# KrishnaswamyLab/MELD

Hardware: AMD Instinct MI355X
Metric: cells/sec through MELD.fit_transform (kNN+Chebyshev) (higher is better)
Workload: dtype f64

## Files before the change

### meld_amd/csrc/knn16.hip

```cpp
#include "common.hpp"

#include <hip/hip_fp16.h>

#include <algorithm>

namespace meld {

constexpr int K16_TS = 64;
constexpr int K16_BQ = 256;
constexpr int K16_THREADS = 256;
constexpr int K16_NWAVE = K16_THREADS / 64;
constexpr int K16_SLACK = 128;
constexpr int K16_CAPMAX = 256;
constexpr int K16_BOUNDS_THREADS = 1024;
constexpr int K16_SLOTS = K16_CAPMAX / 64;
constexpr int K16_DMAX = 16 * 9 - 3;

constexpr int K16_SPLIT_DA = 13;
__host__ __device__ inline void k16_slot(int c, int d, int dA, int* coord, int* piece) {
  *coord = -1;
  *piece = -1;
  if (dA == 0) {
    if (c < d) *coord = c;
    else if (c < d + 3) *piece = 3 + (c - d);
    return;
  }
  const int nb = d - dA;
  if (c < dA) *coord = c;
  else if (c < dA + 3) *piece = c - dA;
  else if (c < 16) return;
  else if (c < 16 + nb) *coord = dA + (c - 16);
  else if (c < 16 + nb + 3) *piece = 3 + (c - 16 - nb);
}

typedef float f32x16 __attribute__((ext_vector_type(16)));
typedef _Float16 f16x8 __attribute__((ext_vector_type(8)));

__device__ __forceinline__ float min3f(float a, float b, float c) { return __builtin_fminf(__builtin_fminf(a, b), c); }
__device__ __forceinline__ float min16(const f32x16& v) {
  const float a = min3f(v[0], v[1], v[2]);
  const float b = min3f(v[3], v[4], v[5]);
  const float c = min3f(v[6], v[7], v[8]);
  const float d = min3f(v[9], v[10], v[11]);
  const float e = min3f(v[12], v[13], v[14]);
  return __builtin_fminf(min3f(a, b, v[15]), min3f(c, d, e));
}

__device__ __forceinline__ unsigned ordered_bits(float f) {
  const unsigned b = __float_as_uint(f);
  return (b & 0x80000000u) ? ~b : (b | 0x80000000u);
}

__device__ __forceinline__ float ld_sc1_f(const float* p) {
  return __hip_atomic_load(p, __ATOMIC_RELAXED, __HIP_MEMORY_SCOPE_AGENT);
}
__device__ __forceinline__ int ld_sc1_i(const int* p) {
  return __hip_atomic_load(p, __ATOMIC_RELAXED, __HIP_MEMORY_SCOPE_AGENT);
}

#define K16_COLD_REGION_END() __builtin_amdgcn_s_waitcnt(0x0F70)

__device__ __forceinline__ bool knn16_row_slot(int p, int n0, int n1, int half, int* q) {
  if (p < half) {
    *q = p;
    return p < n0;
  }
  *q = n0 + (p - half);
  return (p - half) < n1;
}
__device__ __forceinline__ int knn16_split_pos(int pos, int m0, int half) { return pos < m0 ? pos : half + (pos - m0); }

__device__ __forceinline__ float from_ordered_bits(unsigned k) {
  return __uint_as_float((k & 0x80000000u) ? (k & 0x7fffffffu) : ~k);
}

__device__ float knn16_squeeze_row(int n0, int n1, int half, int ksel, int knn1, float rf2, float err, float nq_row,
                                   float* __restrict__ d2row, int* __restrict__ idxrow, int lane, int* n0_out,
                                   int* n1_out, float* r_out) {
  asm volatile("s_waitcnt vmcnt(0)" ::: "memory");
  float d[K16_SLOTS];
  int ix[K16_SLOTS];
  unsigned key[K16_SLOTS];
  bool valid[K16_SLOTS];
#pragma unroll
  for (int e = 0; e < K16_SLOTS; ++e) {
    const int p = lane + 64 * e;
    int q;
    valid[e] = p < 2 * half && knn16_row_slot(p, n0, n1, half, &q);
    if (valid[e]) {
      d[e] = ld_sc1_f(d2row + p);
      ix[e] = ld_sc1_i(idxrow + p);
      key[e] = ordered_bits(d[e]);
    } else {
      d[e] = INFINITY;
      ix[e] = 0x7fffffff;
      key[e] = 0xffffffffu;
    }
  }
  unsigned T = 0;
#pragma unroll 1
  for (int bit = 31; bit >= 0; --bit) {
    const unsigned trial = T | (1u << bit);
    int c = 0;
#pragma unroll
    for (int e = 0; e < K16_SLOTS; ++e) c += __popcll(__ballot(key[e] < trial));
    if (c < ksel) T = trial;
  }
  float R = INFINITY;
  if (knn1 > 0 && n0 + n1 >= knn1) {
    unsigned A = 0;
#pragma unroll 1
    for (int bit = 31; bit >= 0; --bit) {
      const unsigned trial = A | (1u << bit);
      int c = 0;
#pragma unroll
      for (int e = 0; e < K16_SLOTS; ++e) c += __popcll(__ballot(key[e] < trial));
      if (c < knn1) A = trial;
    }
    R = (rf2 * ((from_ordered_bits(A) + nq_row) + err) + err) * 1.00001f + 1e-30f - nq_row;
  }
  *r_out = R;
  const unsigned Tc = min(T, ordered_bits(R));
  int total = 0;
#pragma unroll
  for (int e = 0; e < K16_SLOTS; ++e) total += __popcll(__ballot(valid[e] && key[e] <= Tc));
  const int m0 = (total + 1) >> 1;
  int base = 0;
  float thr = INFINITY;
#pragma unroll
  for (int e = 0; e < K16_SLOTS; ++e) {
    const bool keep = valid[e] && key[e] <= Tc;
    const unsigned long long b = __ballot(keep);
    if (keep) {
      const int dst = knn16_split_pos(base + __popcll(b & ((1ull << lane) - 1ull)), m0, half);
      d2row[dst] = d[e];
      idxrow[dst] = ix[e];
    }
    base += __popcll(b);
    const unsigned long long bt = __ballot(valid[e] && key[e] == T);
    if (bt) thr = __shfl(d[e], __ffsll((long long)bt) - 1, 64);
  }
  *n0_out = m0;
  *n1_out = total - m0;
  return thr;
}

__device__ void knn16_rank_row(int n0, int n1, int half, int ksel, float out_scale, float add, int split_m0,
                               float* __restrict__ d2row, int* __restrict__ idxrow, float* sd, int* si, int lane) {
  asm volatile("s_waitcnt vmcnt(0)" ::: "memory");
  const int n = n0 + n1;
  float d[K16_SLOTS];
  int ix[K16_SLOTS];
  bool valid[K16_SLOTS];
#pragma unroll
  for (int e = 0; e < K16_SLOTS; ++e) {
    const int p = lane + 64 * e;
    int q = 0;
    valid[e] = p < 2 * half && knn16_row_slot(p, n0, n1, half, &q);
    if (valid[e]) {
      d[e] = ld_sc1_f(d2row + p);
      ix[e] = ld_sc1_i(idxrow + p);
      sd[q] = d[e];
      si[q] = ix[e];
    } else {
      d[e] = INFINITY;
      ix[e] = 0x7fffffff;
    }
  }
  asm volatile("s_waitcnt lgkmcnt(0)" ::: "memory");
  int rk[K16_SLOTS];
#pragma unroll
  for (int q = 0; q < K16_SLOTS; ++q) rk[q] = 0;
  for (int e = 0; e < n; ++e) {
    const float de = sd[e];
    const int ie = si[e];
#pragma unroll
    for (int q = 0; q < K16_SLOTS; ++q) rk[q] += (de < d[q] || (de == d[q] && ie < ix[q])) ? 1 : 0;
  }
#pragma unroll
  for (int q = 0; q < K16_SLOTS; ++q) {
    if (valid[q] && rk[q] < ksel) {
      const int dst = split_m0 < 0 ? rk[q] : knn16_split_pos(rk[q], split_m0, half);
      d2row[dst] = (d[q] + add) * out_scale;
      idxrow[dst] = ix[q];
    }
  }
  asm volatile("s_waitcnt lgkmcnt(0)" ::: "memory");
}

__device__ __forceinline__ int k16_scan_tile(int s, int t0, int n_scan, int two_sided) {
  int off = s;
  if (two_sided && s >= K16_BQ / K16_TS) {
    const int j = s - K16_BQ / K16_TS;
    off = (j & 1) ? -1 - (j >> 1) : K16_BQ / K16_TS + (j >> 1);
  }
  const int t = t0 + off;
  return t >= n_scan ? t - n_scan : (t < 0 ? t + n_scan : t);
}

struct K16Args {
  const _Float16* Q16;
  const float* Qn;
  const _Float16* Rt16;
  const float* scale_info;
  int n_ref, n_tiles, ksel, cap;
  const __half* lb2;
  const float* norm2_max;
  float err_coef;
  int tile_origin, batch_every, batch_slack, two_sided;
  unsigned long long* stats;
  const float* thr_init;
  int knn1;
  float rf2, err_c, err_l;
  int* cand_idx;
  float* cand_d2;
  int* cand_cnt;
  float* cand_thr;
  unsigned long long* tiles_done;
  const int* block_order;
  const unsigned* step_list;
  const int* step_cnt;
  long long list_stride;
  int ee_hi;
  int planes_used;
  int count_go;
};
#define K16_COLD(FIELD) \
  (((const volatile K16Args __attribute__((address_space(4)))*)__builtin_amdgcn_kernarg_segment_ptr())->FIELD)

__host__ __device__ constexpr int k16_waves(int KB, int NPROD, bool EE) {
  return ((NPROD == 1 && KB <= 4) ? 3 : ((KB <= 5 || (NPROD == 1 && KB <= 8)) ? 2 : 1)) + ((EE && KB <= 4) ? 1 : 0);
}

template <int KB, int STATS, int NPROD, bool LIST = false, bool EE = false>
__global__ __launch_bounds__(K16_THREADS)
__attribute__((amdgpu_waves_per_eu(k16_waves(KB, NPROD, EE), k16_waves(KB, NPROD, EE)))) void knn16_topk_kernel(const K16Args a) {
  const _Float16* __restrict__ Q16 = a.Q16;
  const float* __restrict__ Qn = a.Qn;
  const _Float16* __restrict__ Rt16 = a.Rt16;
  const int n_tiles = a.n_tiles, ksel = a.ksel, cap = a.cap;
  const __half* __restrict__ lb2 = LIST ? nullptr : a.lb2;
  const int batch_every = a.batch_every, two_sided = a.two_sided;
  int* __restrict__ cand_idx = a.cand_idx;
  float* __restrict__ cand_d2 = a.cand_d2;
  constexpr int TILE_H = KB * 2 * 2 * K16_TS * 8;
  constexpr int TILE_V4 = TILE_H / 8;
  constexpr int LDS_TILE_H = (NPROD == 3) ? TILE_H : TILE_H / 2;
  constexpr bool PAIR = EE;
  constexpr int NBUF = PAIR ? 4 : 3;
  __shared__ __attribute__((aligned(16))) _Float16 lds_ring[NBUF * LDS_TILE_H];
  constexpr int TILE_LDS_BYTES = LDS_TILE_H * 2;
  __shared__ float lds_sd[K16_NWAVE][K16_CAPMAX];
  __shared__ int lds_si[K16_NWAVE][K16_CAPMAX];
  unsigned long long (*lds_wlive)[K16_NWAVE];
  if constexpr (!LIST) {
    __shared__ unsigned long long lds_wlive_own[3][K16_NWAVE];
    lds_wlive = lds_wlive_own;
  } else {
    lds_wlive = reinterpret_cast<unsigned long long (*)[K16_NWAVE]>(&lds_sd[0][0]);
  }

  const int tid = threadIdx.x;
  const int lane = tid & 63;
  const int wave = __builtin_amdgcn_readfirstlane(tid >> 6);
  const int jq = lane & 31;
  const int h = lane >> 5;
  const int bx = a.block_order ? __builtin_amdgcn_readfirstlane(a.block_order[blockIdx.y]) : (int)blockIdx.y;
  const int q_base = bx * K16_BQ + wave * 64;
  int sl_n_ = (int)gridDim.x;
  asm volatile("" : "+s"(sl_n_));
  const int sl_n = sl_n_, sl_y = (int)blockIdx.x;
  typedef const __attribute__((address_space(4))) unsigned* k16_list_ptr;
  const k16_list_ptr my_list = LIST ? (k16_list_ptr)(uintptr_t)(a.step_list + (size_t)bx * (size_t)a.list_stride) : (k16_list_ptr)0;
  const int n_scan = ((LIST ? __builtin_amdgcn_readfirstlane(a.step_cnt[bx]) : n_tiles) - sl_y + sl_n - 1) / sl_n;
  auto list_entry = [&](int s_) __attribute__((always_inline)) { return s_ < n_scan ? my_list[sl_y + sl_n * s_] : 0u; };
  auto entry_live = [&](unsigned e) __attribute__((always_inline)) { return ((e >> (24 + wave)) & 1u) != 0u; };
  const int row_base = (int)(blockIdx.x * (gridDim.y * K16_BQ)) + q_base;
  float* const wave_d2 = cand_d2 + (size_t)row_base * cap;
  int* const wave_idx = cand_idx + (size_t)row_base * cap;

  f16x8 bhi[2][KB], blo[2][KB];
#pragma unroll
  for (int g = 0; g < 2; ++g) {
    const f16x8* qrow = reinterpret_cast<const f16x8*>(Q16 + (size_t)(q_base + g * 32 + jq) * (KB * 32));
#pragma unroll
    for (int kb = 0; kb < KB; ++kb) {
      bhi[g][kb] = qrow[(kb * 2 + h) * 2 + 0];
      if (NPROD == 3) blo[g][kb] = qrow[(kb * 2 + h) * 2 + 1];
    }
  }
  const float* const wave_qn = Qn + q_base;

  int cnt[2] = {0, 0};
  const int half = cap >> 1;
  if (!LIST && lane == 0) lds_wlive[0][wave] = lds_wlive[1][wave] = lds_wlive[2][wave] = ~0ull;
  auto thr_start = [&](int g) __attribute__((always_inline)) { return a.thr_init ? a.thr_init[q_base + g * 32 + jq] : INFINITY; };
  float thrp[2] = {thr_start(0) - wave_qn[jq], thr_start(1) - wave_qn[32 + jq]};
  float ee_c[2] = {0.0f, 0.0f};
  if constexpr (EE) {
    const int ee_hi = a.ee_hi;
    const float s_ = a.scale_info[0];
    const float delta = 3.814697265625e-06f * (a.norm2_max[0] * s_ * s_) + 1e-30f;
#pragma unroll
    for (int g = 0; g < 2; ++g) {
      float qb = 0.0f;
#pragma unroll
      for (int kb = 1; kb < KB; ++kb) {
#pragma unroll
        for (int e = 0; e < 8; ++e) {
          const float v = (16 * kb + 8 * h + e < ee_hi) ? (float)bhi[g][kb][e] : 0.0f;
          qb = fmaf(v, v, qb);
        }
      }
      qb += __shfl_xor(qb, 32, 64);
      ee_c[g] = qb * 1.0001f + delta;
    }
  }
  float wmax = INFINITY;
  if (a.thr_init) {
    float w = fmaxf(thr_start(0), thr_start(1));
#pragma unroll
    for (int off = 32; off > 0; off >>= 1) w = fmaxf(w, __shfl_xor(w, off, 64));
    wmax = w;
  }
  unsigned st_go = 0;
  unsigned st_slow = 0, st_app = 0, st_sq = 0;
  unsigned tm_seg = 0, tm_sel = 0, tm_tail = 0, tm_dma = 0, tm_bar = 0, tm_idle = 0, tm_mark = 0;
  auto tm_now = [&]() __attribute__((always_inline)) { return STATS ? (unsigned)__builtin_readcyclecounter() : 0u; };
  auto tm_lap = [&](unsigned& acc) __attribute__((always_inline)) {
    if (STATS) {
      const unsigned n = tm_now();
      acc += n - tm_mark;
      tm_mark = n;
    }
  };

  const float prune_margin = lb2 ? a.err_coef * a.norm2_max[0] * a.scale_info[0] * a.scale_info[0] : 0.0f;
  const int t0 = (int)((((long long)a.tile_origin + (long long)bx * (K16_BQ / K16_TS)) / sl_n) % n_scan);
  const __half* my_lb = lb2 ? lb2 + (size_t)(bx * K16_NWAVE + wave) * n_tiles : nullptr;
  auto tile_of = [&](int s) { return k16_scan_tile(s, t0, n_scan, two_sided) * sl_n + sl_y; };
  int win_base = 0;
  float win_lb = 0.0f;
  unsigned long long win_rem = 0, my_live = ~0ull;
  auto load_window = [&](int base) __attribute__((always_inline)) {
    const int ss = base + lane;
    win_base = base;
    win_lb = ss < n_scan ? __half2float(my_lb[tile_of(ss)]) : INFINITY;
    win_rem = __ballot(ss < n_scan);
    asm volatile("" : "+v"(win_lb));
  };
  if (my_lb) {
    load_window(0);
    win_rem &= ~1ull;
  }
  auto lds_union = [&](int buf) __attribute__((always_inline)) {
    unsigned lo = 0, hi = 0;
#pragma unroll
    for (int w = 0; w < K16_NWAVE; ++w) {
      const uint2 v = *reinterpret_cast<const uint2*>(&lds_wlive[buf][w]);
      lo |= v.x;
      hi |= v.y;
    }
    return ((unsigned long long)(unsigned)__builtin_amdgcn_readfirstlane((int)hi) << 32) |
           (unsigned long long)(unsigned)__builtin_amdgcn_readfirstlane((int)lo);
  };

  const float4* R4 = reinterpret_cast<const float4*>(Rt16);
  int r4_lo_v, r4_hi_v;
  asm volatile("v_mov_b32 %0, %2\n\tv_mov_b32 %1, %3"
               : "=v"(r4_lo_v), "=v"(r4_hi_v)
               : "s"((int)(unsigned)reinterpret_cast<size_t>(R4)), "s"((int)(reinterpret_cast<size_t>(R4) >> 32)));
  constexpr int N_STAGE = (NPROD == 3) ? KB * 256 : KB * 128;
  constexpr int NS = (N_STAGE + K16_THREADS - 1) / K16_THREADS;
  constexpr bool STAGE_TAIL = (N_STAGE % K16_THREADS) != 0;
  static_assert(NS <= 9, "tile too large for the staging rounds");
  const int stage_off = (NPROD == 3) ? tid : (((tid >> 6) << 7) + (tid & 63));
  constexpr int STAGE_STRIDE = (NPROD == 3) ? K16_THREADS : 2 * K16_THREADS;
  const bool stage_last = !STAGE_TAIL || wave < (N_STAGE % K16_THREADS) / 64;
  const int tail_plane = (NS - 1) * (K16_THREADS / 64) + wave;
  const bool skip_tail = NPROD == 1 && NS >= 2 && tail_plane < 2 * KB && tail_plane >= a.planes_used;
  if (skip_tail) {
#pragma unroll
    for (int b = 0; b < NBUF; ++b)
      reinterpret_cast<float4*>(lds_ring + b * LDS_TILE_H)[((NS - 1) * (K16_THREADS / 64) + wave) * 64 + lane] = make_float4(0.f, 0.f, 0.f, 0.f);
  }
#define K16_ROUND_OK(U) (((U) + 1 < NS || stage_last) && !((U) + 1 == NS && skip_tail))
  const int stage_voff = stage_off * 16;
  typedef __attribute__((address_space(3))) void* lds_ptr_t;
  typedef int k16_i32x4 __attribute__((ext_vector_type(4)));
  const unsigned ring_addr = (unsigned)(size_t)(lds_ptr_t)lds_ring + (unsigned)wave * 1024u;
#define K16_DMA(U, DSTB)                                                                                              \
  asm volatile("s_mov_b32 m0, %0\n\ts_nop 0\n\tbuffer_load_dwordx4 %1, %2, %3 offen lds" ::"s"(__builtin_amdgcn_readfirstlane(    \
                   (int)(ring_addr + (DSTB) + (unsigned)((U) * K16_THREADS * 16)))),                                   \
               "v"(stage_voff), "s"(rsrc), "s"((U) * STAGE_STRIDE * 16)                                                \
               : "memory")
#define K16_LOAD(TILE, DSTB)                                                                                       \
  do {                                                                                                             \
    const size_t src_ = (((size_t)(unsigned)__builtin_amdgcn_readfirstlane(r4_hi_v) << 32) |                       \
                         (size_t)(unsigned)__builtin_amdgcn_readfirstlane(r4_lo_v)) +                              \
                        (size_t)(TILE) * (TILE_V4 * 16);                                                           \
    const k16_i32x4 rsrc = {(int)(unsigned)src_, (int)((src_ >> 32) & 0xffffu), TILE_V4 * 16, 0x00020000};         \
    if constexpr (NS > 0) if (K16_ROUND_OK(0)) K16_DMA(0, DSTB);                                                   \
    if constexpr (NS > 1) if (K16_ROUND_OK(1)) K16_DMA(1, DSTB);                                                   \
    if constexpr (NS > 2) if (K16_ROUND_OK(2)) K16_DMA(2, DSTB);                                                   \
    if constexpr (NS > 3) if (K16_ROUND_OK(3)) K16_DMA(3, DSTB);                                                   \
    if constexpr (NS > 4) if (K16_ROUND_OK(4)) K16_DMA(4, DSTB);                                                   \
    if constexpr (NS > 5) if (K16_ROUND_OK(5)) K16_DMA(5, DSTB);                                                   \
    if constexpr (NS > 6) if (K16_ROUND_OK(6)) K16_DMA(6, DSTB);                                                   \
    if constexpr (NS > 7) if (K16_ROUND_OK(7)) K16_DMA(7, DSTB);                                                   \
    if constexpr (NS > 8) if (K16_ROUND_OK(8)) K16_DMA(8, DSTB);                                                   \
  } while (0)
#define K16_STAGED() __builtin_amdgcn_s_waitcnt(0x0F70)
  constexpr int N_INFLIGHT = NS - (STAGE_TAIL ? 1 : 0);
  constexpr int N_INFLIGHT_SKIP = (!STAGE_TAIL && NS >= 2) ? N_INFLIGHT - 1 : N_INFLIGHT;
#define K16_STAGED_BUT_LAST()                                                                                      \
  do {                                                                                                             \
    if (skip_tail) __builtin_amdgcn_s_waitcnt(0x0F70 | (N_INFLIGHT_SKIP & 15) | ((N_INFLIGHT_SKIP >> 4) << 14));   \
    else __builtin_amdgcn_s_waitcnt(0x0F70 | (N_INFLIGHT & 15) | ((N_INFLIGHT >> 4) << 14));                       \
  } while (0)
#define K16_TILE_BARRIER() asm volatile("s_waitcnt lgkmcnt(0)\n\ts_barrier" ::: "memory")
  if constexpr (!PAIR) K16_LOAD(__builtin_amdgcn_readfirstlane(LIST ? (int)(list_entry(0) & 0xFFFFFFu) : tile_of(0)), 0u);

#pragma unroll
  for (int g = 0; g < 2; ++g) {
#pragma unroll
    for (int kb = 0; kb < KB; ++kb) {
      asm volatile("" : "+v"(bhi[g][kb]));
      if (NPROD == 3) asm volatile("" : "+v"(blo[g][kb]));
    }
    asm volatile("" : "+v"(thrp[g]));
  }

  f32x16 accA0, accA1, accB0, accB1;
#pragma unroll
  for (int r = 0; r < 16; ++r) accB0[r] = accB1[r] = INFINITY;
  int refB = 0;

  auto mfma_block = [&](const _Float16* tile, int sub, f32x16& c0, f32x16& c1) __attribute__((always_inline)) {
#pragma unroll
    for (int r = 0; r < 16; ++r) c0[r] = c1[r] = 0.0f;
    const f16x8* a8 = reinterpret_cast<const f16x8*>(tile) + sub * 32 + jq;
#pragma unroll
    for (int kb = 0; kb < KB; ++kb) {
      const f16x8 ahi = NPROD == 3 ? a8[((kb * 2 + h) * 2 + 0) * K16_TS] : a8[(kb * 2 + h) * K16_TS];
      c0 = __builtin_amdgcn_mfma_f32_32x32x16_f16(ahi, bhi[0][kb], c0, 0, 0, 0);
      c1 = __builtin_amdgcn_mfma_f32_32x32x16_f16(ahi, bhi[1][kb], c1, 0, 0, 0);
      if (NPROD == 3) {
        const f16x8 alo = a8[((kb * 2 + h) * 2 + 1) * K16_TS];
        c0 = __builtin_amdgcn_mfma_f32_32x32x16_f16(ahi, blo[0][kb], c0, 0, 0, 0);
        c1 = __builtin_amdgcn_mfma_f32_32x32x16_f16(ahi, blo[1][kb], c1, 0, 0, 0);
        c0 = __builtin_amdgcn_mfma_f32_32x32x16_f16(alo, bhi[0][kb], c0, 0, 0, 0);
        c1 = __builtin_amdgcn_mfma_f32_32x32x16_f16(alo, bhi[1][kb], c1, 0, 0, 0);
      }
    }
  };
  auto vote = [&](const f32x16& c0, const f32x16& c1, float& m0, float& m1) __attribute__((always_inline)) {
    m0 = min16(c0);
    m1 = min16(c1);
  };
  auto squeeze = [&](int g, int j) __attribute__((always_inline)) {
    const int cg = g ? cnt[1] : cnt[0];
    const int n0 = __shfl(cg, j, 64), n1 = __shfl(cg, j + 32, 64);
    const size_t ro = (size_t)(g * 32 + j) * cap;
    int m0, m1;
    float rcut = INFINITY, err = 0.0f;
    const int knn1 = K16_COLD(knn1);
    const float nq_row = wave_qn[g * 32 + j];
    if (knn1 > 0) {
      const float* sinfo = K16_COLD(scale_info);
      const float nmax_s = K16_COLD(norm2_max)[0] * sinfo[0] * sinfo[0];
      err = (K16_COLD(err_c) * nmax_s + K16_COLD(err_l) * sqrtf(nq_row * nmax_s)) * 1.001f;
    }
    float nt = knn16_squeeze_row(n0, n1, half, ksel, knn1, K16_COLD(rf2), err, nq_row, wave_d2 + ro, wave_idx + ro, lane, &m0, &m1, &rcut);
    if (m0 > half - 32) {
      knn16_rank_row(m0, m1, half, ksel, 1.0f, 0.0f, (min(m0 + m1, ksel) + 1) >> 1, wave_d2 + ro, wave_idx + ro, lds_sd[wave],
                     lds_si[wave], lane);
      const int tot = min(m0 + m1, ksel);
      m0 = (tot + 1) >> 1;
      m1 = tot - m0;
      asm volatile("s_waitcnt vmcnt(0)" ::: "memory");
      nt = ld_sc1_f(wave_d2 + ro + knn16_split_pos(tot - 1, m0, half));
    }
    if (jq == j) {
      const int mine = h ? m1 : m0;
      if (g) cnt[1] = mine; else cnt[0] = mine;
      const float t_list = (n0 + n1 >= ksel) ? nt : INFINITY;
      thrp[g] = fminf(thrp[g], fminf(t_list, rcut));
    }
    asm volatile("" : "+v"(thrp[0]), "+v"(thrp[1]), "+v"(cnt[0]), "+v"(cnt[1]));
  };
  auto refresh_wmax = [&]() __attribute__((always_inline)) {
    if (my_lb == nullptr) return;
    float w = fmaxf(thrp[0] + wave_qn[jq], thrp[1] + wave_qn[32 + jq]);
#pragma unroll
    for (int off = 32; off > 0; off >>= 1) w = fmaxf(w, __shfl_xor(w, off, 64));
    wmax = w;
  };
  auto select = [&](const f32x16& c0, const f32x16& c1, float m0, float m1, int ref_base) __attribute__((always_inline)) {
    unsigned long long need = 0;
    if (STATS) ++st_slow;
#pragma unroll
    for (int g = 0; g < 2; ++g) {
      const f32x16 acc = g ? c1 : c0;
      if (!__any((g ? m1 : m0) < thrp[g])) continue;
      const unsigned rowoff4 = (unsigned)((g * 32 + jq) * cap + h * half) * 4u;
      auto append = [&](int r) __attribute__((always_inline)) {
        const float v = acc[r];
        if (v < thrp[g]) {
          const unsigned off4 = rowoff4 + 4u * (unsigned)(g ? cnt[1]++ : cnt[0]++);
          if (STATS) ++st_app;
          *reinterpret_cast<float*>(reinterpret_cast<char*>(wave_d2) + off4) = v;
          *reinterpret_cast<int*>(reinterpret_cast<char*>(wave_idx) + off4) = ref_base + (r & 3) + 8 * (r >> 2);
        }
      };
#pragma unroll
      for (int t = 0; t < 5; ++t) {
        if (__any(min3f(acc[3 * t], acc[3 * t + 1], acc[3 * t + 2]) < thrp[g])) {
          append(3 * t);
          append(3 * t + 1);
          append(3 * t + 2);
        }
      }
      if (__any(acc[15] < thrp[g])) append(15);
      const unsigned long long full = __ballot((g ? cnt[1] : cnt[0]) > half - 16);
      need |= ((full | (full >> 32)) & 0xffffffffull) << (32 * g);
    }
    if (__builtin_expect(need != 0, 0)) {
      while (need) {
        const int j = __ffsll((long long)need) - 1;
        need &= need - 1;
        squeeze(j >> 5, j & 31);
        if (STATS) ++st_sq;
      }
      refresh_wmax();
      K16_COLD_REGION_END();
    }
  };
  constexpr int N_MFMA = 2 * KB * (NPROD == 3 ? 3 : 1);
  constexpr int N_DSR = KB * (NPROD == 3 ? 2 : 1);
  constexpr int VALU_PER_MFMA = (N_MFMA >= 16) ? 1 : ((N_MFMA >= 8) ? 2 : 4);
  auto pipeline_order = [&]() __attribute__((always_inline)) {
    if (NPROD == 3) {
      __builtin_amdgcn_sched_group_barrier(0x100, N_DSR, 0);
      __builtin_amdgcn_sched_group_barrier(0x002, 4, 0);
#pragma unroll
      for (int i = 0; i < N_MFMA; ++i) {
        __builtin_amdgcn_sched_group_barrier(0x008, 1, 0);
        __builtin_amdgcn_sched_group_barrier(0x002, VALU_PER_MFMA, 0);
      }
    } else {
      constexpr int A_AHEAD = 4;
      __builtin_amdgcn_sched_group_barrier(0x100, KB < A_AHEAD ? KB : A_AHEAD, 0);
      __builtin_amdgcn_sched_group_barrier(0x002, 4, 0);
#pragma unroll
      for (int kb = 0; kb < KB; ++kb) {
        __builtin_amdgcn_sched_group_barrier(0x008, 1, 0);
        __builtin_amdgcn_sched_group_barrier(0x002, VALU_PER_MFMA, 0);
        __builtin_amdgcn_sched_group_barrier(0x008, 1, 0);
        __builtin_amdgcn_sched_group_barrier(0x002, VALU_PER_MFMA, 0);
        if (kb + A_AHEAD < KB) __builtin_amdgcn_sched_group_barrier(0x100, 1, 0);
      }
    }
  };
  auto segment = [&](const _Float16* tile, int sub, f32x16& n0, f32x16& n1, const f32x16& c0, const f32x16& c1, int ref_base, bool issue,
                     bool fresh) __attribute__((always_inline)) {
    if (issue) mfma_block(tile, sub, n0, n1);
    float m0, m1;
    vote(c0, c1, m0, m1);
    if (issue) asm volatile("" : "+v"(m0), "+v"(m1));
    const bool hit = m0 < thrp[0] || m1 < thrp[1];
    if (issue) pipeline_order();
    if (fresh && __any(hit)) {
      unsigned t0s = tm_now();
      select(c0, c1, m0, m1, ref_base);
      if (STATS) {
        const unsigned d = tm_now() - t0s;
        tm_sel += d;
        tm_mark += d;
      }
    }
  };

  auto next_step = [&](int after, int par_, bool* live) __attribute__((always_inline)) {
    if (!my_lb) {
      *live = true;
      return after + 1;
    }
    unsigned long long any = lds_union(par_) & win_rem;
    if (__builtin_expect(any == 0, 0)) {
      while (any == 0 && win_base + 64 < n_scan) {
        load_window(win_base + 64);
        my_live = __ballot(win_lb <= wmax + prune_margin);
        if (lane == 0) lds_wlive[2][wave] = my_live;
        __syncthreads();
        any = lds_union(2) & win_rem;
        __syncthreads();
      }
      K16_COLD_REGION_END();
    }
    if (any == 0) {
      *live = false;
      return n_scan;
    }
    const int i = (int)__ffsll((long long)any) - 1;
    *live = (my_live >> i) & 1ull;
    win_rem &= ~((2ull << i) - 1ull);
    return win_base + i;
  };

  int n_done = 0;
  auto ee_tile = [&](const _Float16* tile_r, int t) __attribute__((always_inline)) {
    const f16x8* a8 = reinterpret_cast<const f16x8*>(tile_r) + jq;
    const f16x8 aA = a8[h * K16_TS], aB = a8[32 + h * K16_TS];
    const float tA0 = thrp[0] + ee_c[0], tA1 = thrp[1] + ee_c[1];
#pragma unroll
    for (int sub = 0; sub < 2; ++sub) {
#pragma unroll
      for (int r = 0; r < 16; ++r) accA0[r] = accA1[r] = 0.0f;
      accA0 = __builtin_amdgcn_mfma_f32_32x32x16_f16(sub ? aB : aA, bhi[0][0], accA0, 0, 0, 0);
      accA1 = __builtin_amdgcn_mfma_f32_32x32x16_f16(sub ? aB : aA, bhi[1][0], accA1, 0, 0, 0);
      if (__any(min16(accA0) < tA0 || min16(accA1) < tA1)) {
        const f16x8* as = a8 + sub * 32;
#pragma unroll
        for (int kb = 1; kb < KB; ++kb) {
          const f16x8 ahi = as[(kb * 2 + h) * K16_TS];
          accA0 = __builtin_amdgcn_mfma_f32_32x32x16_f16(ahi, bhi[0][kb], accA0, 0, 0, 0);
          accA1 = __builtin_amdgcn_mfma_f32_32x32x16_f16(ahi, bhi[1][kb], accA1, 0, 0, 0);
        }
        const float m0 = min16(accA0), m1 = min16(accA1);
        if (__any(m0 < thrp[0] || m1 < thrp[1])) {
          const unsigned t0s = tm_now();
          select(accA0, accA1, m0, m1, t * K16_TS + 32 * sub + 4 * h);
          if (STATS) {
            const unsigned dsel = tm_now() - t0s;
            tm_sel += dsel;
            tm_mark += dsel;
          }
        }
        ++st_go;
      }
    }
    ++n_done;
  };
  int s_cur = 0;
  int par = 0;
  int it = 0;
  bool live_cur = true;
  bool pend = false;
  unsigned e_pref = 0u;
  int t_cur = tile_of(0);
  bool live_next = true;
  int s_next = next_step(0, 0, &live_next);
  int t_next = s_next < n_scan ? tile_of(s_next) : t_cur;
  if constexpr (LIST) {
    const unsigned e0 = list_entry(0), e1 = list_entry(1);
    e_pref = list_entry(2);
    t_cur = (int)(e0 & 0xFFFFFFu);
    live_cur = entry_live(e0);
    s_next = 1;
    t_next = s_next < n_scan ? (int)(e1 & 0xFFFFFFu) : t_cur;
    live_next = entry_live(e1);
  }
  if constexpr (!PAIR) {
    if (s_next < n_scan) {
      K16_LOAD(__builtin_amdgcn_readfirstlane(t_next), (unsigned)TILE_LDS_BYTES);
// ... 192 lines not shown
__global__ __launch_bounds__(256) __attribute__((amdgpu_waves_per_eu(WPE, WPE))) void knn16_partial_filter_kernel(const _Float16* __restrict__ Q16, const float* __restrict__ Qn,
                                                                   const _Float16* __restrict__ Rt16, const float* __restrict__ scale_info,
                                                                   const float* __restrict__ norm2_max, const float* __restrict__ thr_init,
                                                                   unsigned* step_list, const int* __restrict__ step_cnt, long long list_stride,
                                                                   int* __restrict__ cnt_out, unsigned long long* __restrict__ tested,
                                                                   const int* __restrict__ block_order, int KB, int ee_hi) {
  static_assert(TPS >= 2 && TPS <= 32 && (TPS & 1) == 0, "tiles per step");
  __shared__ __attribute__((aligned(16))) _Float16 ring[2][TPS][2 * K16_TS * 8];
  __shared__ unsigned wmask[2][4];
  const int tid = threadIdx.x, lane = tid & 63;
  const int wave = __builtin_amdgcn_readfirstlane(tid >> 6);
  const int jq = lane & 31, h = lane >> 5;
  const int bx = block_order ? __builtin_amdgcn_readfirstlane(block_order[blockIdx.x]) : (int)blockIdx.x;
  const int q_base = bx * K16_BQ + wave * 64;
  f16x8 b0[2];
  float tA[2];
  {
    const float s_ = scale_info[0];
    const float delta = 3.814697265625e-06f * (norm2_max[0] * s_ * s_) + 1e-30f;
#pragma unroll
    for (int g = 0; g < 2; ++g) {
      const int q = q_base + g * 32 + jq;
      const f16x8* qrow = reinterpret_cast<const f16x8*>(Q16 + (size_t)q * (size_t)(KB * 32));
      b0[g] = qrow[h * 2];
      float qb = 0.0f;
      for (int kb = 1; kb < KB; ++kb) {
        const f16x8 v8 = qrow[(kb * 2 + h) * 2];
#pragma unroll
        for (int e = 0; e < 8; ++e) {
          const float v = (16 * kb + 8 * h + e < ee_hi) ? (float)v8[e] : 0.0f;
          qb = fmaf(v, v, qb);
        }
      }
      qb += __shfl_xor(qb, 32, 64);
      tA[g] = (thr_init[q] - Qn[q]) + (qb * 1.0001f + delta);
    }
  }
  unsigned* const my_list_w = step_list + (size_t)bx * (size_t)list_stride;
  const int n = __builtin_amdgcn_readfirstlane(step_cnt[bx]);
  const int n_steps = (n + TPS - 1) / TPS;
  const size_t tile_bytes = (size_t)KB * 4096;
  const int plane_stride = 2048;
  const size_t src_base = reinterpret_cast<size_t>(Rt16);
  typedef __attribute__((address_space(3))) void* lds_ptr_t;
  typedef int i32x4 __attribute__((ext_vector_type(4)));
  const unsigned ring_base = (unsigned)(size_t)(lds_ptr_t)&ring[0][0][0];
  const int lane16 = lane * 16;
  auto load_entries = [&](int step) __attribute__((always_inline)) {
    const int idx = step * TPS + lane;
    return (lane < TPS && idx < n) ? my_list_w[idx] : 0u;
  };
  auto stage = [&](unsigned ev, int buf) __attribute__((always_inline)) {
#pragma unroll
    for (int u = 0; u < TPS / 2; ++u) {
      const int k = wave * (TPS / 2) + u;
      const unsigned e = (unsigned)__builtin_amdgcn_readlane((int)ev, k >> 1);
      if (e >> 24) {
        const size_t src = src_base + (size_t)(e & 0xFFFFFFu) * tile_bytes;
        const i32x4 rsrc = {(int)(unsigned)src, (int)((src >> 32) & 0xffffu), 4096, 0x00020000};
        asm volatile("s_mov_b32 m0, %0\n\ts_nop 0\n\tbuffer_load_dwordx4 %1, %2, %3 offen lds" ::"s"(__builtin_amdgcn_readfirstlane(
                         (int)(ring_base + (unsigned)((buf * TPS + (k >> 1)) * 2048 + (k & 1) * 1024)))),
                     "v"(lane16), "s"(rsrc), "s"((k & 1) * plane_stride)
                     : "memory");
      }
    }
  };
  int out_n = 0;
  unsigned long long n_tested = 0;
  auto emit = [&](unsigned ev, int par) __attribute__((always_inline)) {
    unsigned nm = 0u;
#pragma unroll
    for (int w = 0; w < 4; ++w) nm |= ((wmask[par][w] >> lane) & 1u) << w;
    nm &= (ev >> 24);
    const bool keep = nm != 0u;
    const unsigned long long b = __ballot(keep);
    if (keep) my_list_w[out_n + __popcll(b & ((1ull << lane) - 1ull))] = (ev & 0xFFFFFFu) | (nm << 24);
    out_n += __popcll(b);
  };
  unsigned ev_prev = 0u, ev_cur = load_entries(0), ev_nxt = load_entries(1);
  if (n_steps > 0) stage(ev_cur, 0);
  __builtin_amdgcn_s_waitcnt(0x0F70);
  asm volatile("s_waitcnt lgkmcnt(0)\n\ts_barrier" ::: "memory");
  for (int s = 0; s < n_steps; ++s) {
    const int buf = s & 1;
    const unsigned ev_nn = load_entries(s + 2);
    if (s + 1 < n_steps) stage(ev_nxt, buf ^ 1);
    if (wave == 0 && s > 0) emit(ev_prev, buf ^ 1);
    unsigned mybits = 0u;
#pragma unroll
    for (int j = 0; j < TPS; ++j) {
      const unsigned e = (unsigned)__builtin_amdgcn_readlane((int)ev_cur, j);
      if ((e >> (24 + wave)) & 1u) {
        const f16x8* a8 = reinterpret_cast<const f16x8*>(&ring[buf][j][0]) + jq;
        const f16x8 aA = a8[h * K16_TS], aB = a8[h * K16_TS + 32];
        f32x16 c00, c01, c10, c11;
#pragma unroll
        for (int r = 0; r < 16; ++r) c00[r] = c01[r] = c10[r] = c11[r] = 0.0f;
        c00 = __builtin_amdgcn_mfma_f32_32x32x16_f16(aA, b0[0], c00, 0, 0, 0);
        c01 = __builtin_amdgcn_mfma_f32_32x32x16_f16(aA, b0[1], c01, 0, 0, 0);
        c10 = __builtin_amdgcn_mfma_f32_32x32x16_f16(aB, b0[0], c10, 0, 0, 0);
        c11 = __builtin_amdgcn_mfma_f32_32x32x16_f16(aB, b0[1], c11, 0, 0, 0);
        const bool hit = __builtin_fminf(min16(c00), min16(c10)) < tA[0] || __builtin_fminf(min16(c01), min16(c11)) < tA[1];
        if (__any(hit)) mybits |= 1u << j;
        ++n_tested;
      }
    }
    if (lane == 0) wmask[buf][wave] = mybits;
    __builtin_amdgcn_s_waitcnt(0x0F70);
    asm volatile("s_waitcnt lgkmcnt(0)\n\ts_barrier" ::: "memory");
    ev_prev = ev_cur;
    ev_cur = ev_nxt;
    ev_nxt = ev_nn;
  }
  if (wave == 0) {
    if (n_steps > 0) emit(ev_prev, (n_steps - 1) & 1);
    if (lane == 0) cnt_out[bx] = out_n;
  }
  if (tested && lane == 0) atomicAdd(tested, n_tested);
}

template <int SL>
__device__ __forceinline__ void k16_bitonic_sort(unsigned long long (&key)[SL], int lane) {
  constexpr int NE = 64 * SL;
#pragma unroll
  for (int k = 2; k <= NE; k <<= 1) {
#pragma unroll
    for (int j = k >> 1; j > 0; j >>= 1) {
      if (j >= 64) {
        const int je = j >> 6;
#pragma unroll
        for (int e = 0; e < SL; ++e) {
          if ((e & je) == 0) {
            const int i = 64 * e + lane;
            const bool asc = (i & k) == 0;
            const unsigned long long a = key[e], b = key[e | je];
            const bool sw = asc ? (b < a) : (a < b);
            key[e] = sw ? b : a;
            key[e | je] = sw ? a : b;
          }
        }
      } else {
#pragma unroll
        for (int e = 0; e < SL; ++e) {
          const int i = 64 * e + lane;
          const unsigned long long o = __shfl_xor(key[e], j, 64);
          const bool keep_min = ((i & j) == 0) == ((i & k) == 0);
          key[e] = keep_min ? (o < key[e] ? o : key[e]) : (o < key[e] ? key[e] : o);
        }
      }
    }
  }
}
template <int SL>
__device__ __forceinline__ void k16_finish_row(float* __restrict__ drow, int* __restrict__ irow, int n0, int half, int n_all, int n,
                                               float add, float out_scale, int lane) {
  unsigned long long key[SL];
#pragma unroll
  for (int e = 0; e < SL; ++e) {
    const int i = lane + 64 * e;
    const int p = i < n0 ? i : half + (i - n0);
    key[e] = ~0ull;
    if (i < n_all) key[e] = ((unsigned long long)ordered_bits(drow[p] + 0.0f) << 32) | (unsigned)irow[p];
  }
  k16_bitonic_sort<SL>(key, lane);
#pragma unroll
  for (int e = 0; e < SL; ++e) {
    const int i = 64 * e + lane;
    if (i < n) {
      drow[i] = (from_ordered_bits((unsigned)(key[e] >> 32)) + add) * out_scale;
      irow[i] = (int)(unsigned)key[e];
    }
  }
}
__global__ __launch_bounds__(256) void knn16_finish_rows_kernel(float* __restrict__ d2, int* __restrict__ idx,
                                                                int* __restrict__ cnt, const float* __restrict__ Qn,
                                                                const float* __restrict__ scale_info, int64_t n_rows,
                                                                int64_t q_pad, int cap, int ksel) {
  const int lane = threadIdx.x & 63;
  const int64_t row = (int64_t)blockIdx.x * 4 + (threadIdx.x >> 6);
  if (row >= n_rows) return;
  const int packed = cnt[row];
  const int n0 = packed & 0xffff, n1 = (packed >> 16) & 0xffff, half = cap >> 1;
  float* drow = d2 + (size_t)row * cap;
  int* irow = idx + (size_t)row * cap;
  const int n_all = n0 + n1, n = min(n_all, ksel);
  const float add = Qn[row % q_pad], out_scale = scale_info[1];
  if (n_all <= 64)
    k16_finish_row<1>(drow, irow, n0, half, n_all, n, add, out_scale, lane);
  else if (n_all <= 128)
    k16_finish_row<2>(drow, irow, n0, half, n_all, n, add, out_scale, lane);
  else
    k16_finish_row<K16_SLOTS>(drow, irow, n0, half, n_all, n, add, out_scale, lane);
  if (lane == 0) cnt[row] = n;
}

constexpr int K16_MERGE_MAX = 4096;
constexpr int K16_MERGE_SLOTS = K16_MERGE_MAX / 64;

__global__ __launch_bounds__(64) void knn16_merge_slices_kernel(const int* __restrict__ s_idx,
                                                                const float* __restrict__ s_d2,
                                                                const int* __restrict__ s_cnt, int q_count, int q_pad,
                                                                int ksel, int cap, int n_slices,
                                                                int* __restrict__ out_idx, float* __restrict__ out_d2,
                                                                int* __restrict__ out_cnt) {
  extern __shared__ __attribute__((aligned(16))) unsigned char merge_lds[];
  float* sd = reinterpret_cast<float*>(merge_lds);
  int* si = reinterpret_cast<int*>(merge_lds) + n_slices * ksel;
  const int lane = threadIdx.x;
  const int q = blockIdx.x;
  if (q >= q_count) return;
  int n = 0;
  for (int s = 0; s < n_slices; ++s) {
    const int row = s * q_pad + q;
    const int c = min(s_cnt[row], ksel);
    for (int e = lane; e < c; e += 64) {
      sd[n + e] = s_d2[(size_t)row * cap + e];
      si[n + e] = s_idx[(size_t)row * cap + e];
    }
    n += c;
  }
  __syncthreads();
  for (int p = lane; p < n; p += 64) {
    const float dp = sd[p];
    const int ip = si[p];
    int rk = 0;
    for (int e = 0; e < n; ++e) rk += (sd[e] < dp || (sd[e] == dp && si[e] < ip)) ? 1 : 0;
    if (rk < ksel) {
      out_d2[(size_t)q * cap + rk] = dp;
      out_idx[(size_t)q * cap + rk] = ip;
    }
  }
  if (lane == 0) out_cnt[q] = min(n, ksel);
}

__device__ __forceinline__ void k16_tile_sphere(const float* xs_dyn, int ld, int cnt, int d, int KB, int dA, int tile,
                                                _Float16* __restrict__ cent16, float* __restrict__ cent_n, float* __restrict__ cent_r) {
#define XS(r, k) xs_dyn[(r) * ld + (k)]
  __shared__ float cs[K16_DMAX + 19];
  const int tid = threadIdx.x;
  if (tid < KB * 16) {
    float acc = 0.0f;
    if (tid < d)
      for (int r = 0; r < cnt; ++r) acc += XS(r, tid);
    cs[tid] = tid < d ? acc / (float)cnt : 0.0f;
  }
  __syncthreads();
  __shared__ float cb[K16_DMAX + 19];
  __shared__ float s_best_r2;
  if (tid < 64) {
    const int lane = tid;
    auto far2 = [&](int* who) {
      float r2 = -1.0f;
      if (lane < cnt) {
        r2 = 0.0f;
        int k = 0;
        for (; k + 8 <= d; k += 8) {
          float t[8];
#pragma unroll
          for (int u = 0; u < 8; ++u) t[u] = XS(lane, k + u) - cs[k + u];
#pragma unroll
          for (int u = 0; u < 8; ++u) r2 = fmaf(t[u], t[u], r2);
        }
        for (; k < d; ++k) {
          const float t = XS(lane, k) - cs[k];
          r2 = fmaf(t, t, r2);
        }
      }
      auto dppf = [](float old, float v, auto ctrl, auto rows) __attribute__((always_inline)) {
        return __int_as_float(__builtin_amdgcn_update_dpp(__float_as_int(old), __float_as_int(v), decltype(ctrl)::value, decltype(rows)::value, 0xF, false));
      };
      using std::integral_constant;
      float m = r2;
      m = fmaxf(m, dppf(m, m, integral_constant<int, 0xB1>{}, integral_constant<int, 0xF>{}));
      m = fmaxf(m, dppf(m, m, integral_constant<int, 0x4E>{}, integral_constant<int, 0xF>{}));
      m = fmaxf(m, dppf(m, m, integral_constant<int, 0x141>{}, integral_constant<int, 0xF>{}));
      m = fmaxf(m, dppf(m, m, integral_constant<int, 0x140>{}, integral_constant<int, 0xF>{}));
      m = fmaxf(m, dppf(m, m, integral_constant<int, 0x142>{}, integral_constant<int, 0xA>{}));
      m = fmaxf(m, dppf(m, m, integral_constant<int, 0x143>{}, integral_constant<int, 0xC>{}));
      m = __int_as_float(__builtin_amdgcn_readlane(__float_as_int(m), 63));
      *who = __ffsll((long long)__ballot(r2 == m)) - 1;
      return m;
    };
    float best = INFINITY;
    constexpr int MEB_STEPS = 24;
    for (int it = 1; it <= MEB_STEPS + 1; ++it) {
      int who;
      const float r2 = far2(&who);
      if (r2 < best) {
        best = r2;
        for (int k = lane; k < KB * 16; k += 64) cb[k] = cs[k];
      }
      if (it <= MEB_STEPS) {
        const float wgt = 1.0f / (float)(it + 1);
        for (int k = lane; k < d; k += 64) cs[k] = fmaf(wgt, XS(who, k) - cs[k], cs[k]);
      }
      __builtin_amdgcn_s_waitcnt(0xC07F);
      asm volatile("" ::: "memory");
    }
    for (int k = lane; k < KB * 16; k += 64) cs[k] = cb[k];
    if (lane == 0) s_best_r2 = best;
  }
  __syncthreads();
  if (tid < 64) {
    const float r2 = s_best_r2;
    float n = 0.0f;
    for (int k = 0; k < d; ++k) n = fmaf(cs[k], cs[k], n);
    if (tid == 0) {
      cent_r[tile] = sqrtf(r2) * 1.0001f + 1e-30f;
      cent_n[tile] = n;
    }
  } else if (tid - 64 < KB * 2) {
    const int g = tid - 64;
    f16x8 hi, lo;
#pragma unroll
    for (int e = 0; e < 8; ++e) {
      int cc, pc;
      k16_slot(g * 8 + e, d, dA, &cc, &pc);
      _Float16 h16 = (_Float16)0.0f, l16 = (_Float16)0.0f;
      if (cc >= 0) {
        h16 = (_Float16)cs[cc];
        l16 = (_Float16)(cs[cc] - (float)h16);
      } else if (pc >= 0) {
        h16 = (_Float16)1.0f;
      }
      hi[e] = h16;
      lo[e] = l16;
    }
    f16x8* qrow = reinterpret_cast<f16x8*>(cent16) + (size_t)tile * ((size_t)KB * 4);
    qrow[g * 2 + 0] = hi;
    qrow[g * 2 + 1] = lo;
  }
#undef XS
}

__global__ __launch_bounds__(256) void tile_spheres_kernel(const double* __restrict__ X, int64_t N, int d,
                                                           const double* __restrict__ mean,
                                                           const float* __restrict__ scale_info, int KB,
                                                           _Float16* __restrict__ cent16, float* __restrict__ cent_n,
                                                           float* __restrict__ cent_r, int tile0, int dA) {
  extern __shared__ float xs_dyn[];
  const int ld = d | 1;
  const int tid = threadIdx.x;
  const int tile = tile0 + (int)blockIdx.x;
  const int64_t row0 = (int64_t)tile * K16_TS;
  const int cnt = (int)min((int64_t)K16_TS, N - row0);
// ... 1429 lines not shown
```

Measured before the change: 28.54 million.

## Interleave kNN candidate distance and index into 8-byte records

Candidate buffers switch from separate distance and index arrays to interleaved 8-byte {d2, idx} records spread across the two existing allocations per wave. Appends, squeeze, rank and finish each do one 64-bit load or store per candidate instead of two 32-bit ones. The finish kernel is rewritten to read the interleaved layout and adds a block barrier before writing sorted rows back in place. This is meant to cut memory instructions and transactions in the top-k candidate path, at the cost of more intricate addressing whose correctness depends on row grouping and cap assumptions.

```diff
diff --git a/meld_amd/csrc/knn16.hip b/meld_amd/csrc/knn16.hip
--- a/meld_amd/csrc/knn16.hip
+++ b/meld_amd/csrc/knn16.hip
@@ -51,15 +51,31 @@
   return (b & 0x80000000u) ? ~b : (b | 0x80000000u);
 }
 
-__device__ __forceinline__ float ld_sc1_f(const float* p) {
-  return __hip_atomic_load(p, __ATOMIC_RELAXED, __HIP_MEMORY_SCOPE_AGENT);
-}
-__device__ __forceinline__ int ld_sc1_i(const int* p) {
-  return __hip_atomic_load(p, __ATOMIC_RELAXED, __HIP_MEMORY_SCOPE_AGENT);
-}
 
 #define K16_COLD_REGION_END() __builtin_amdgcn_s_waitcnt(0x0F70)
 
+struct __attribute__((aligned(8))) K16Rec {
+  float d2;
+  int idx;
+};
+static_assert(sizeof(K16Rec) == 8, "a candidate entry is one 8-byte record");
+__device__ __forceinline__ unsigned k16_half_stride(int cap) { return 32u * 4u * (unsigned)cap; }
+static_assert(64ull * K16_CAPMAX * 4ull + 8ull * K16_CAPMAX < (1ull << 32), "lane offsets within a wave's rows are 32 bits");
+__device__ __forceinline__ K16Rec* k16_rec_at(char* row0, int p, int half, unsigned hstride) {
+  unsigned off = p < half ? 8u * (unsigned)p : hstride + 8u * (unsigned)(p - half);
+  asm volatile("" : "+v"(off));
+  return reinterpret_cast<K16Rec*>(row0 + off);
+}
+__device__ __forceinline__ K16Rec ld_sc1_rec(const K16Rec* p) {
+  const unsigned long long v = __hip_atomic_load(reinterpret_cast<const unsigned long long*>(p), __ATOMIC_RELAXED, __HIP_MEMORY_SCOPE_AGENT);
+  K16Rec r;
+  r.d2 = __uint_as_float((unsigned)v);
+  r.idx = (int)(unsigned)(v >> 32);
+  return r;
+}
+__device__ __forceinline__ void st_rec(K16Rec* p, float d2, int idx) {
+  *reinterpret_cast<uint2*>(p) = make_uint2(__float_as_uint(d2), (unsigned)idx);
+}
 __device__ __forceinline__ bool knn16_row_slot(int p, int n0, int n1, int half, int* q) {
   if (p < half) {
     *q = p;
@@ -75,7 +91,7 @@
 }
 
 __device__ float knn16_squeeze_row(int n0, int n1, int half, int ksel, int knn1, float rf2, float err, float nq_row,
-                                   float* __restrict__ d2row, int* __restrict__ idxrow, int lane, int* n0_out,
+                                   char* __restrict__ row0, unsigned hstride, int lane, int* n0_out,
                                    int* n1_out, float* r_out) {
   asm volatile("s_waitcnt vmcnt(0)" ::: "memory");
   float d[K16_SLOTS];
@@ -88,8 +104,9 @@
     int q;
     valid[e] = p < 2 * half && knn16_row_slot(p, n0, n1, half, &q);
     if (valid[e]) {
-      d[e] = ld_sc1_f(d2row + p);
-      ix[e] = ld_sc1_i(idxrow + p);
+      const K16Rec rec = ld_sc1_rec(k16_rec_at(row0, p, half, hstride));
+      d[e] = rec.d2;
+      ix[e] = rec.idx;
       key[e] = ordered_bits(d[e]);
     } else {
       d[e] = INFINITY;
@@ -133,8 +150,7 @@
     const unsigned long long b = __ballot(keep);
     if (keep) {
       const int dst = knn16_split_pos(base + __popcll(b & ((1ull << lane) - 1ull)), m0, half);
-      d2row[dst] = d[e];
-      idxrow[dst] = ix[e];
+      st_rec(k16_rec_at(row0, dst, half, hstride), d[e], ix[e]);
     }
     base += __popcll(b);
     const unsigned long long bt = __ballot(valid[e] && key[e] == T);
@@ -146,7 +162,7 @@
 }
 
 __device__ void knn16_rank_row(int n0, int n1, int half, int ksel, float out_scale, float add, int split_m0,
-                               float* __restrict__ d2row, int* __restrict__ idxrow, float* sd, int* si, int lane) {
+                               char* __restrict__ row0, unsigned hstride, float* sd, int* si, int lane) {
   asm volatile("s_waitcnt vmcnt(0)" ::: "memory");
   const int n = n0 + n1;
   float d[K16_SLOTS];
@@ -158,8 +174,9 @@
     int q = 0;
     valid[e] = p < 2 * half && knn16_row_slot(p, n0, n1, half, &q);
     if (valid[e]) {
-      d[e] = ld_sc1_f(d2row + p);
-      ix[e] = ld_sc1_i(idxrow + p);
+      const K16Rec rec = ld_sc1_rec(k16_rec_at(row0, p, half, hstride));
+      d[e] = rec.d2;
+      ix[e] = rec.idx;
       sd[q] = d[e];
       si[q] = ix[e];
     } else {
@@ -181,8 +198,7 @@
   for (int q = 0; q < K16_SLOTS; ++q) {
     if (valid[q] && rk[q] < ksel) {
       const int dst = split_m0 < 0 ? rk[q] : knn16_split_pos(rk[q], split_m0, half);
-      d2row[dst] = (d[q] + add) * out_scale;
-      idxrow[dst] = ix[q];
+      st_rec(k16_rec_at(row0, dst, half, hstride), (d[q] + add) * out_scale, ix[q]);
     }
   }
   asm volatile("s_waitcnt lgkmcnt(0)" ::: "memory");
@@ -241,8 +257,8 @@
   const int n_tiles = a.n_tiles, ksel = a.ksel, cap = a.cap;
   const __half* __restrict__ lb2 = LIST ? nullptr : a.lb2;
   const int batch_every = a.batch_every, two_sided = a.two_sided;
-  int* __restrict__ cand_idx = a.cand_idx;
-  float* __restrict__ cand_d2 = a.cand_d2;
+  int* const cand_idx = a.cand_idx;
+  float* const cand_d2 = a.cand_d2;
   constexpr int TILE_H = KB * 2 * 2 * K16_TS * 8;
   constexpr int TILE_V4 = TILE_H / 8;
   constexpr int LDS_TILE_H = (NPROD == 3) ? TILE_H : TILE_H / 2;
@@ -276,8 +292,8 @@
   auto list_entry = [&](int s_) __attribute__((always_inline)) { return s_ < n_scan ? my_list[sl_y + sl_n * s_] : 0u; };
   auto entry_live = [&](unsigned e) __attribute__((always_inline)) { return ((e >> (24 + wave)) & 1u) != 0u; };
   const int row_base = (int)(blockIdx.x * (gridDim.y * K16_BQ)) + q_base;
-  float* const wave_d2 = cand_d2 + (size_t)row_base * cap;
-  int* const wave_idx = cand_idx + (size_t)row_base * cap;
+  char* const wave_rec0 = reinterpret_cast<char*>(cand_idx + (size_t)row_base * cap);
+  char* const wave_rec1 = reinterpret_cast<char*>(cand_d2 + (size_t)row_base * cap);
 
   f16x8 bhi[2][KB], blo[2][KB];
 #pragma unroll
@@ -461,7 +477,8 @@
   auto squeeze = [&](int g, int j) __attribute__((always_inline)) {
     const int cg = g ? cnt[1] : cnt[0];
     const int n0 = __shfl(cg, j, 64), n1 = __shfl(cg, j + 32, 64);
-    const size_t ro = (size_t)(g * 32 + j) * cap;
+    char* const row0 = (g ? wave_rec1 : wave_rec0) + (unsigned)(j * cap) * 4u;
+    const unsigned hstride = k16_half_stride(cap);
     int m0, m1;
     float rcut = INFINITY, err = 0.0f;
     const int knn1 = K16_COLD(knn1);
@@ -471,15 +488,14 @@
       const float nmax_s = K16_COLD(norm2_max)[0] * sinfo[0] * sinfo[0];
       err = (K16_COLD(err_c) * nmax_s + K16_COLD(err_l) * sqrtf(nq_row * nmax_s)) * 1.001f;
     }
-    float nt = knn16_squeeze_row(n0, n1, half, ksel, knn1, K16_COLD(rf2), err, nq_row, wave_d2 + ro, wave_idx + ro, lane, &m0, &m1, &rcut);
+    float nt = knn16_squeeze_row(n0, n1, half, ksel, knn1, K16_COLD(rf2), err, nq_row, row0, hstride, lane, &m0, &m1, &rcut);
     if (m0 > half - 32) {
-      knn16_rank_row(m0, m1, half, ksel, 1.0f, 0.0f, (min(m0 + m1, ksel) + 1) >> 1, wave_d2 + ro, wave_idx + ro, lds_sd[wave],
-                     lds_si[wave], lane);
+      knn16_rank_row(m0, m1, half, ksel, 1.0f, 0.0f, (min(m0 + m1, ksel) + 1) >> 1, row0, hstride, lds_sd[wave], lds_si[wave], lane);
       const int tot = min(m0 + m1, ksel);
       m0 = (tot + 1) >> 1;
       m1 = tot - m0;
       asm volatile("s_waitcnt vmcnt(0)" ::: "memory");
-      nt = ld_sc1_f(wave_d2 + ro + knn16_split_pos(tot - 1, m0, half));
+      nt = ld_sc1_rec(k16_rec_at(row0, knn16_split_pos(tot - 1, m0, half), half, hstride)).d2;
     }
     if (jq == j) {
       const int mine = h ? m1 : m0;
@@ -503,14 +519,16 @@
     for (int g = 0; g < 2; ++g) {
       const f32x16 acc = g ? c1 : c0;
       if (!__any((g ? m1 : m0) < thrp[g])) continue;
-      const unsigned rowoff4 = (unsigned)((g * 32 + jq) * cap + h * half) * 4u;
+      const unsigned rowoff = (unsigned)(lane * cap) * 4u;
+      char* const rec_base = g ? wave_rec1 : wave_rec0;
       auto append = [&](int r) __attribute__((always_inline)) {
         const float v = acc[r];
         if (v < thrp[g]) {
-          const unsigned off4 = rowoff4 + 4u * (unsigned)(g ? cnt[1]++ : cnt[0]++);
+          const unsigned off = rowoff + 8u * (unsigned)(g ? cnt[1]++ : cnt[0]++);
           if (STATS) ++st_app;
-          *reinterpret_cast<float*>(reinterpret_cast<char*>(wave_d2) + off4) = v;
-          *reinterpret_cast<int*>(reinterpret_cast<char*>(wave_idx) + off4) = ref_base + (r & 3) + 8 * (r >> 2);
+          float v_lo;
+          asm volatile("v_mov_b32 %0, %1" : "=v"(v_lo) : "v"(v));
+          st_rec(reinterpret_cast<K16Rec*>(rec_base + off), v_lo, ref_base + ((r & 3) + 8 * (r >> 2)));
         }
       };
 #pragma unroll
@@ -1009,45 +1027,57 @@
   }
 }
 template <int SL>
-__device__ __forceinline__ void k16_finish_row(float* __restrict__ drow, int* __restrict__ irow, int n0, int half, int n_all, int n,
-                                               float add, float out_scale, int lane) {
-  unsigned long long key[SL];
-#pragma unroll
-  for (int e = 0; e < SL; ++e) {
+__device__ __forceinline__ void k16_sort_head(unsigned long long (&key)[K16_SLOTS], int lane) {
+  unsigned long long k[SL];
+#pragma unroll
+  for (int e = 0; e < SL; ++e) k[e] = key[e];
+  k16_bitonic_sort<SL>(k, lane);
+#pragma unroll
+  for (int e = 0; e < SL; ++e) key[e] = k[e];
+}
+__global__ __launch_bounds__(256) void knn16_finish_rows_kernel(float* d2, int* idx, int* __restrict__ cnt, const float* __restrict__ Qn,
+                                                                const float* __restrict__ scale_info, int64_t n_rows,
+                                                                int64_t q_pad, int cap, int ksel) {
+  if ((int64_t)blockIdx.x * 4 >= n_rows) return;
+  const int lane = threadIdx.x & 63;
+  const int wv = threadIdx.x >> 6;
+  const int64_t pair = (int64_t)blockIdx.x * 2 + (wv >> 1);
+  const int g = wv & 1, j = (int)(pair & 31);
+  const int64_t slot0 = (pair >> 5) * 64 + j;
+  const int64_t row = slot0 + 32 * g;
+  const int packed = cnt[row];
+  const int n0 = packed & 0xffff, n1 = (packed >> 16) & 0xffff;
+  const char* row0 = (g ? reinterpret_cast<const char*>(d2) : reinterpret_cast<const char*>(idx)) + (size_t)slot0 * cap * 4;
+  const unsigned hstride = k16_half_stride(cap);
+  float* drow = d2 + (size_t)row * cap;
+  int* irow = idx + (size_t)row * cap;
+  const int n_all = n0 + n1, n = min(n_all, ksel);
+  const float add = Qn[row % q_pad], out_scale = scale_info[1];
+  unsigned long long key[K16_SLOTS];
+#pragma unroll
+  for (int e = 0; e < K16_SLOTS; ++e) {
     const int i = lane + 64 * e;
-    const int p = i < n0 ? i : half + (i - n0);
     key[e] = ~0ull;
-    if (i < n_all) key[e] = ((unsigned long long)ordered_bits(drow[p] + 0.0f) << 32) | (unsigned)irow[p];
-  }
-  k16_bitonic_sort<SL>(key, lane);
-#pragma unroll
-  for (int e = 0; e < SL; ++e) {
+    if (i < n_all) {
+      const uint2 rec = *reinterpret_cast<const uint2*>(row0 + (i < n0 ? 8u * (unsigned)i : hstride + 8u * (unsigned)(i - n0)));
+      key[e] = ((unsigned long long)ordered_bits(__uint_as_float(rec.x) + 0.0f) << 32) | rec.y;
+    }
+  }
+  if (n_all <= 64)
+    k16_sort_head<1>(key, lane);
+  else if (n_all <= 128)
+    k16_sort_head<2>(key, lane);
+  else
+    k16_sort_head<K16_SLOTS>(key, lane);
+  __syncthreads();
+#pragma unroll
+  for (int e = 0; e < K16_SLOTS; ++e) {
     const int i = 64 * e + lane;
     if (i < n) {
       drow[i] = (from_ordered_bits((unsigned)(key[e] >> 32)) + add) * out_scale;
       irow[i] = (int)(unsigned)key[e];
     }
   }
-}
-__global__ __launch_bounds__(256) void knn16_finish_rows_kernel(float* __restrict__ d2, int* __restrict__ idx,
-                                                                int* __restrict__ cnt, const float* __restrict__ Qn,
-                                                                const float* __restrict__ scale_info, int64_t n_rows,
-                                                                int64_t q_pad, int cap, int ksel) {
-  const int lane = threadIdx.x & 63;
-  const int64_t row = (int64_t)blockIdx.x * 4 + (threadIdx.x >> 6);
-  if (row >= n_rows) return;
-  const int packed = cnt[row];
-  const int n0 = packed & 0xffff, n1 = (packed >> 16) & 0xffff, half = cap >> 1;
-  float* drow = d2 + (size_t)row * cap;
-  int* irow = idx + (size_t)row * cap;
-  const int n_all = n0 + n1, n = min(n_all, ksel);
-  const float add = Qn[row % q_pad], out_scale = scale_info[1];
-  if (n_all <= 64)
-    k16_finish_row<1>(drow, irow, n0, half, n_all, n, add, out_scale, lane);
-  else if (n_all <= 128)
-    k16_finish_row<2>(drow, irow, n0, half, n_all, n, add, out_scale, lane);
-  else
-    k16_finish_row<K16_SLOTS>(drow, irow, n0, half, n_all, n, add, out_scale, lane);
   if (lane == 0) cnt[row] = n;
 }
 
```

Result: no change. 28.78 million, median of 6 (+0.8%).
